# brucechin/OctopusZK

Hardware: AMD Instinct MI355X
Metric: BN254 G1 VariableBaseMSM Mscalar-mul/s at 2^20 (higher is better)
Workload: dtype u32; 1 GPU; VariableBaseMSM BN254 G1 2^20 random scalars/bases per GPU, bit-exact vs the serial CPU path (BASELINE.json configs[1]); n_per_gpu=1048576, window_bits=16, windows=8, glv=True, prepared_bases=False, msms_in_flight=3, schedule=pipeline3, parallelism=index-range shard x1, RCCL all-gather of 192-B partials + HIP point sum

## Files before the change

octopuszk_amd/csrc/ec_fft.cuh:

```cuda
#pragma once
#include "points_scale.cuh"

namespace ozk {

template <class CV>
OZK_HD void ec_write2(const Jac<CV>& a, const Jac<CV>& b, bool negate_b, u32* oa, u32* ob) {
  using IO = CurveIO<CV>;
  const bool ia = is_inf(a), ib = is_inf(b);
  if (ia || ib) {
    IO::template write<WireIn>(a, oa);
    if (ib) return IO::template write_inf<WireIn>(ob);
    return IO::template write_jac<WireIn>(b, inv(b.Z), negate_b, ob);
  }
  const auto za = reduce_to<32>(a.Z), zb = reduce_to<32>(b.Z);
  const auto ti = inv(mul(za, zb));
  IO::template write_jac<WireIn>(a, mul(ti, zb), false, oa);
  IO::template write_jac<WireIn>(b, mul(ti, za), negate_b, ob);
}
template <class CV>
OZK_HD Aff<typename CV::EA> ec_to_affine(const Jac<CV>& r) {
  using IO = CurveIO<CV>;
  using EA = typename CV::EA;
  Aff<EA> q = IO::aff_infinity();
  if (is_inf(r)) return q;
  q = IO::jac_to_aff(r, inv(r.Z));
  q.x = EA(canonical(q.x));
  q.y = EA(canonical(q.y));
  return q;
}
template <class EA>
OZK_HD Aff<EA> ec_neg(const Aff<EA>& q) {
  Aff<EA> m;
  m.x = q.x;
  m.y = EA(canonical(neg(q.y)));
  return m;
}

template <class CV>
OZK_HD void points_add_one(const u32* pa, const u32* pb, bool negate_b, u32* out) {
  using IO = CurveIO<CV>;
  const auto a = IO::aff_from_wire(pa);
  auto b = IO::aff_from_wire(pb);
  if (negate_b) b = ec_neg(b);
  IO::template write<WireIn>(jac_madd<CV>(from_affine<CV>(a), b), out);
}

struct EcFftTwiddle {
  u32 base[8], k[8];
};
OZK_HD void ecfft_twiddle(const EcFftTwiddle& c, u32 i, u32 (&out)[8]) {
  using F = Fe<FrParams, 32>;
  F acc = F(to_mont<FrParams>(c.k)), b = F(to_mont<FrParams>(c.base));
  for (u32 e = i; e; e >>= 1) {
    if (e & 1) acc = F(mul(acc, b));
    b = F(sqr(b));
  }
  from_mont(acc, out);
}
OZK_HD void ecfft_schedule(const EcFftTwiddle& c, u32 i, bool glv, ScaleSchedule& s) {
  u32 w[8];
  ecfft_twiddle(c, i, w);
  scale_recode(w, glv, s);
}

template <class CV, bool GLV>
OZK_HD void ecfft_butterfly(const u32* pa, const u32* pb, const ScaleSchedule* sa, const ScaleSchedule* sb, u32* oa,
                            u32* ob) {
  auto a = CurveIO<CV>::aff_from_wire(pa);
  const auto b = CurveIO<CV>::aff_from_wire(pb);
  if (sa) a = ec_to_affine<CV>(scale_ladder<CV, GLV>(a, *sa));
  const Jac<CV> v = sb ? scale_ladder<CV, GLV>(b, *sb) : from_affine<CV>(b);
  const Jac<CV> sum = jac_madd<CV>(v, a);
  const Jac<CV> dif = jac_madd<CV>(v, ec_neg(a));
  ec_write2<CV>(sum, dif, true, oa, ob);
}

OZK_HD bool words_are(const u32* w, const u32 (&v)[8]) {
  u32 d = 0;
  for (int i = 0; i < 8; i++) d |= w[i] ^ v[i];
  return d == 0;
}
template <class CV>
OZK_HD Jac<CV> sparse_term(const Jac<CV>& acc, const u32* p, const u32* c) {
  auto q = CurveIO<CV>::aff_from_wire(p);
  if (c) {
    u32 k[8];
    for (int i = 0; i < 8; i++) k[i] = c[i];
    for (int it = 0; it < 6 && mp_geq<8>(k, GlvConsts::R32); it++) mp_sub<8>(k, GlvConsts::R32);
    const u32 one[8] = {1, 0, 0, 0, 0, 0, 0, 0};
    u32 m1[8];
    for (int i = 0; i < 8; i++) m1[i] = GlvConsts::R32[i];
    m1[0] -= 1;
    if (words_are(k, m1)) {
      q = ec_neg(q);
    } else if (!words_are(k, one)) {
      const Jac<CV> v = is_inf(q) ? jac_infinity<CV>() : scalar_mul<CV>(q, k, 8);
      q = ec_to_affine<CV>(v);
    }
  }
  return jac_madd<CV>(acc, q);
}

#if defined(__HIPCC__)
constexpr int EC_LONG = 64;
constexpr int EC_LONG_LANES = 4096;

template <int TYPE>
__global__ __launch_bounds__(64) void k_ecfft_recode(EcFftTwiddle c, int n, ScaleSchedule* out) {
  const int i = blockIdx.x * blockDim.x + threadIdx.x;
  if (i >= n) return;
  ScaleSchedule s;
  ecfft_schedule(c, (u32)i, EcType<TYPE>::GLV, s);
  out[i] = s;
}

template <int TYPE>
__global__ __launch_bounds__(64) void k_ecfft_permute(const u32* __restrict__ in, int n, int logn, u32* __restrict__ out) {
  using CV = typename EcType<TYPE>::CV;
  using IO = CurveIO<CV>;
  constexpr int PW = IO::WIRE_JAC_WORDS;
  const int i = blockIdx.x * blockDim.x + threadIdx.x;
  if (i >= n) return;
  const u32 j = logn ? __brev((u32)i) >> (32 - logn) : 0u;
  IO::template write_aff<WireIn>(IO::aff_from_wire(in + (size_t)PW * i), out + (size_t)PW * j);
}

template <int TYPE>
__global__ __launch_bounds__(64) void k_ecfft_pass(u32* data, int logn, int logh, const ScaleSchedule* tab, int stride,
                                                   int skip0, const ScaleSchedule* sa) {
  using CV = typename EcType<TYPE>::CV;
  constexpr int PW = CurveIO<CV>::WIRE_JAC_WORDS;
  const u32 t = blockIdx.x * blockDim.x + threadIdx.x;
  if (t >= (1u << (logn - 1))) return;
  const int logb = logn - 1 - logh;
  const u32 j = t >> logb, k = t & ((1u << logb) - 1);
  u32* pa = data + (size_t)PW * (((size_t)k << (logh + 1)) + j);
  u32* pb = pa + ((size_t)PW << logh);
  const ScaleSchedule* sb = (j == 0 && skip0) ? nullptr : tab + (size_t)j * stride;
  ecfft_butterfly<CV, EcType<TYPE>::GLV>(pa, pb, sa, sb, pa, pb);
}

template <int TYPE>
__global__ __launch_bounds__(64) void k_points_add(const u32* a, const u32* b, int n, int negate_b, u32* out) {
  using CV = typename EcType<TYPE>::CV;
  constexpr int PW = CurveIO<CV>::WIRE_JAC_WORDS;
  const int i = blockIdx.x * blockDim.x + threadIdx.x;
  if (i >= n) return;
  points_add_one<CV>(a + (size_t)PW * i, b + (size_t)PW * i, negate_b != 0, out + (size_t)PW * i);
}

template <int TYPE>
__global__ __launch_bounds__(64) void k_sparse_points(const u32* __restrict__ ptr, const u32* __restrict__ idx,
                                                      const u32* __restrict__ coeff, const u32* __restrict__ points,
                                                      int rows, u32* __restrict__ out) {
  using CV = typename EcType<TYPE>::CV;
  using IO = CurveIO<CV>;
  constexpr int PW = IO::WIRE_JAC_WORDS;
  const int row = blockIdx.x * blockDim.x + threadIdx.x;
  if (row >= rows) return;
  const u32 b = ptr[row], e = ptr[row + 1];
  if (e - b > (u32)EC_LONG) return;
  Jac<CV> acc = jac_infinity<CV>();
  for (u32 t = b; t < e; t++)
    acc = sparse_term<CV>(acc, points + (size_t)PW * idx[t], coeff ? coeff + (size_t)8 * t : nullptr);
  IO::template write<WireIn>(acc, out + (size_t)PW * row);
}
template <int TYPE>
__global__ __launch_bounds__(64) void k_sparse_points_long(const u32* __restrict__ ptr, const u32* __restrict__ idx,
                                                           const u32* __restrict__ coeff, const u32* __restrict__ points,
                                                           const u32* __restrict__ long_rows, u32* __restrict__ part) {
  using CV = typename EcType<TYPE>::CV;
  using IO = CurveIO<CV>;
  constexpr int PW = IO::WIRE_JAC_WORDS;
  const u32 g = blockIdx.x * blockDim.x + threadIdx.x;
  const u32 lr = g / EC_LONG_LANES, l = g % EC_LONG_LANES;
  const u32 row = long_rows[lr];
  const u32 b = ptr[row], e = ptr[row + 1];
  Jac<CV> acc = jac_infinity<CV>();
  for (u32 t = b + l; t < e; t += EC_LONG_LANES)
    acc = sparse_term<CV>(acc, points + (size_t)PW * idx[t], coeff ? coeff + (size_t)8 * t : nullptr);
  IO::template write<WireIn>(acc, part + (size_t)PW * g);
}
template <int TYPE>
__global__ __launch_bounds__(64) void k_points_sum64(const u32* __restrict__ in, int groups, const u32* __restrict__ dest,
                                                     u32* __restrict__ out) {
  using CV = typename EcType<TYPE>::CV;
  using IO = CurveIO<CV>;
  constexpr int PW = IO::WIRE_JAC_WORDS;
  const int g = blockIdx.x * blockDim.x + threadIdx.x;
  if (g >= groups) return;
  Jac<CV> acc = jac_infinity<CV>();
  for (int i = 0; i < 64; i++) acc = jac_madd<CV>(acc, IO::aff_from_wire(in + (size_t)PW * (64 * (size_t)g + i)));
  IO::template write<WireIn>(acc, out + (size_t)PW * (dest ? dest[g] : (u32)g));
}
#endif

}
```

octopuszk_amd/csrc/glv.cuh:

```cuda
#pragma once
#include "curve.cuh"

namespace ozk {

struct GlvConsts {
  static constexpr u32 R32[8] = {0xf0000001u, 0x43e1f593u, 0x79b97091u, 0x2833e848u, 0x8181585du, 0xb85045b6u, 0xe131a029u, 0x30644e72u};
  static constexpr u32 G1C[3] = {0xc7e0b3d7u, 0xd91d232eu, 0x00000002u};
  static constexpr u32 G2C[5] = {0x391eb18du, 0x7a7bd9d4u, 0xa773d2cfu, 0x4ccef014u, 0x00000002u};
  static constexpr u32 A1[2] = {0x94d213e3u, 0x89d32568u};
  static constexpr u32 A2[4] = {0x1221250bu, 0x0be4e154u, 0xeeb859fdu, 0x6f4d8248u};
  static constexpr u32 B1ABS[4] = {0x7d4f1128u, 0x8211bbebu, 0xeeb859fcu, 0x6f4d8248u};
  static constexpr u32 B2[2] = {0x94d213e3u, 0x89d32568u};
  static constexpr u32 BETA_G1[9] = {0xa337995u, 0x158d1d23u, 0x189c9b98u, 0x12fa4e45u, 0x185faadcu, 0x176f16du, 0xeed93bau, 0x14291140u, 0xc0afeu};
  static constexpr u32 BETA_G2[9] = {0x18ccb791u, 0x175b1c3au, 0xb83d6e2u, 0xe8ed071u, 0x1282bee2u, 0x4220e84u, 0x1fe4017fu, 0x15084d4au, 0x169119u};
};

template <int NA, int NB, int NR>
OZK_HD void mp_mul_lo(const u32* a, const u32* b, u32* r) {
  u64 carry = 0;
#pragma unroll
  for (int k = 0; k < NR; k++) {
    u64 lo = carry & 0xffffffffull;
    u64 hi = carry >> 32;
#pragma unroll
    for (int i = 0; i < NA; i++) {
      const int j = k - i;
      if (j >= 0 && j < NB) {
        const u64 p = (u64)a[i] * b[j];
        lo += p & 0xffffffffull;
        hi += p >> 32;
      }
    }
    r[k] = (u32)lo;
    carry = hi + (lo >> 32);
  }
}
template <int NA, int NB>
OZK_HD void mp_mul(const u32* a, const u32* b, u32* r) { mp_mul_lo<NA, NB, NA + NB>(a, b, r); }

template <int N>
OZK_HD void mp_sub(u32* a, const u32* b) {
  u64 br = 0;
#pragma unroll
  for (int i = 0; i < N; i++) {
    const u64 t = (u64)a[i] - b[i] - br;
    a[i] = (u32)t;
    br = (t >> 32) & 1;
  }
}
template <int N>
OZK_HD bool mp_geq(const u32* a, const u32* b) {
  for (int i = N - 1; i >= 0; i--) {
    if (a[i] > b[i]) return true;
    if (a[i] < b[i]) return false;
  }
  return true;
}
template <int N>
OZK_HD void mp_neg(u32* a) {
  u64 c = 1;
#pragma unroll
  for (int i = 0; i < N; i++) {
    c += (u64)(~a[i]);
    a[i] = (u32)c;
    c >>= 32;
  }
}

OZK_HD void glv_decompose(const u32 (&k_in)[8], u32 (&k1)[4], bool& neg1, u32 (&k2)[4], bool& neg2) {
  u32 k[8];
#pragma unroll
  for (int i = 0; i < 8; i++) k[i] = k_in[i];
  for (int it = 0; it < 6 && mp_geq<8>(k, GlvConsts::R32); it++) mp_sub<8>(k, GlvConsts::R32);
  u32 p1[11], p2[13];
  mp_mul<8, 3>(k, GlvConsts::G1C, p1);
  mp_mul<8, 5>(k, GlvConsts::G2C, p2);
  const u32* c1 = p1 + 8;
  const u32* c2 = p2 + 8;
  u32 t1[5], t2[5], s1[5], s2[5];
  mp_mul_lo<3, 2, 5>(c1, GlvConsts::A1, t1);
  mp_mul_lo<5, 4, 5>(c2, GlvConsts::A2, t2);
#pragma unroll
  for (int i = 0; i < 5; i++) s1[i] = k[i];
  mp_sub<5>(s1, t1);
  mp_sub<5>(s1, t2);
  mp_mul_lo<3, 4, 5>(c1, GlvConsts::B1ABS, s2);
  mp_mul_lo<5, 2, 5>(c2, GlvConsts::B2, t2);
  mp_sub<5>(s2, t2);
  neg1 = (s1[4] >> 31) != 0;
  neg2 = (s2[4] >> 31) != 0;
  if (neg1) mp_neg<5>(s1);
  if (neg2) mp_neg<5>(s2);
#pragma unroll
  for (int i = 0; i < 4; i++) {
    k1[i] = s1[i];
    k2[i] = s2[i];
  }
}

template <class CV>
OZK_HD Fe<FqParams, 16> glv_beta() {
  if constexpr (CurveIO<CV>::CW == 16) return fe_const<FqParams, 16>(GlvConsts::BETA_G2);
  else return fe_const<FqParams, 16>(GlvConsts::BETA_G1);
}
template <class CV>
OZK_HD Aff<typename CV::EA> glv_image(const Aff<typename CV::EA>& q) {
  Aff<typename CV::EA> q2;
  q2.x = typename CV::EA(canonical(scale(q.x, glv_beta<CV>())));
  q2.y = q.y;
  return q2;
}

}
```

octopuszk_amd/csrc/msm_var.cuh:

```cuda
#pragma once
#include "curve.cuh"
#include "glv.cuh"

namespace ozk {

constexpr u32 BID_NONE = 0xffffffffu;

struct MsmPlan {
  int n_in;
  int glv;
  int n;
  int sd;
  int c;
  int cb;
  int W;
  int L1;
  int LK;
  int S;
};

OZK_HD u32 scalar_digit(const u32 (&s)[8], int w, int c) {
  const int bit = w * c;
  const int wi = bit >> 5, sh = bit & 31;
  u32 v = s[wi] >> sh;
// ... 859 lines not shown
    const long long e0 = (s + L < n_in) ? (s + L) : n_in;
    bool any = false;
    for (long long p = s; p < e0; p++) any = any || (bid_in[p] != BID_NONE);
    live = any;
  }
  if (live) {
    const long long e = (s + L < n_in) ? (s + L) : n_in;
    const u32 first_bid = bid_at(s);
    const bool cb = (s > 0) && (bid_at(s - 1) == first_bid) && (first_bid != BID_NONE);
    const u32 last_bid = bid_at(e - 1);
    const bool cf = (e < n_in) && (bid_at(e) == last_bid) && (last_bid != BID_NONE);
    u32 cur = BID_NONE;
    bool cur_cb = false;
    using Acc = std::conditional_t<(FIRST && CV::LDS_ACC), RunAccLds<CV>, RunAcc<CV, FIRST>>;
    Acc acc;
    if constexpr (FIRST && CV::LDS_ACC) {
      extern __shared__ u32 ozk_acc_lds[];
      acc.init(ozk_acc_lds);
    }
    if constexpr (FIRST) {
      const u32 n_e = (u32)(e - s);
      const uint2* ent_c = ent + s;
      const uint2 e_first = ent_c[0];
      uint2 e_next = ent_c[n_e > 1 ? 1 : 0];
      u32 v_cur = e_first.x;
      const __amdgpu_buffer_rsrc_t table = Acc::table_rsrc(pts_in);
      typename Acc::Raw r = Acc::load_raw_buf(table, v_cur);
      u32 b_cur = first_bid;
      for (u32 k = 0; k < n_e; k++) {
        const u32 b = b_cur;
        const bool negate = (v_cur & SIDX_NEG) != 0;
        const auto q = [&] {
          if constexpr (LAZY) return Acc::decode_unsigned(r);
          else return Acc::decode(r, v_cur);
        }();
        const u32 k2 = (k + 2 < n_e) ? k + 2 : n_e - 1;
        const uint2 en = e_next;
        r = Acc::load_raw_buf(table, en.x);
        b_cur = en.y;
        v_cur = en.x;
        e_next = ent_c[k2];
        if (b != cur) {
          if (cur != BID_NONE) {
            if (cur_cb) {
              head_bid = cur;
              acc.store(pts_out + (size_t)(2 * (size_t)t) * IO::REC_WORDS);
            } else {
              acc.store(buckets + (size_t)cur * IO::REC_WORDS);
            }
          }
          cur = b;
          cur_cb = (k == 0) && cb;
          if constexpr (LAZY) acc.start_signed(q, negate);
          else acc.start_q(q);
        } else {
          if constexpr (LAZY) acc.accumulate_signed(q, negate);
          else acc.accumulate_q(q);
        }
      }
    } else {
    for (long long p = s; p < e; p++) {
      const u32 b = bid_in[p];
      if (b != cur) {
        if (cur != BID_NONE) {
          if (cur_cb) {
            head_bid = cur;
            acc.store(pts_out + (size_t)(2 * (size_t)t) * IO::REC_WORDS);
          } else {
            acc.store(buckets + (size_t)cur * IO::REC_WORDS);
          }
        }
        cur = b;
        cur_cb = (p == s) && cb;
        if (b != BID_NONE) acc.start(pts_in, idx_in, p);
      } else if (b != BID_NONE) {
        acc.accumulate(pts_in, idx_in, p);
      }
    }
    }
    if (cur != BID_NONE) {
      if (cur_cb) {
        head_bid = cur;
        acc.store(pts_out + (size_t)(2 * (size_t)t) * IO::REC_WORDS);
        if (cf) {
          tail_bid = cur;
          if constexpr (FIRST) {
            acc.store_infinity(pts_out + (size_t)(2 * (size_t)t + 1) * IO::REC_WORDS);
          } else {
            IO::store_rec_jac(jac_infinity<CV>(), pts_out + (size_t)(2 * (size_t)t + 1) * IO::REC_WORDS);
          }
        }
      } else if (cf) {
        tail_bid = cur;
        acc.store(pts_out + (size_t)(2 * (size_t)t + 1) * IO::REC_WORDS);
      } else {
        acc.store(buckets + (size_t)cur * IO::REC_WORDS);
      }
    }
  }
  bid_out[2 * (size_t)t] = head_bid;
  bid_out[2 * (size_t)t + 1] = tail_bid;
}

template <class CV, bool FIRST, bool LAZY = false>
__global__ void __launch_bounds__(256, (FIRST && CV::LDS_ACC) ? 2 : 1)
k_segreduce(const u32* __restrict__ bid_in, const u32* __restrict__ idx_in, const u32* __restrict__ pts_in,
            const u32* __restrict__ d_count, int n_in_static, int L,
            u32* __restrict__ buckets, u32* __restrict__ bid_out, u32* __restrict__ pts_out,
            int n_lanes, unsigned long long* __restrict__ clk) {
  const int t = blockIdx.x * blockDim.x + threadIdx.x;
  unsigned long long w0 = 0, c0 = 0;
  if constexpr (FIRST) {
    if (clk != nullptr && threadIdx.x == 0) {
      w0 = (unsigned long long)wall_clock64();
      c0 = (unsigned long long)clock64();
      atomicMax(&clk[0], ~w0);
    }
  }
  if (t < n_lanes)
    segreduce_lane<CV, FIRST, LAZY>(t, bid_in, idx_in, pts_in, d_count, n_in_static, L, buckets, bid_out, pts_out);
  if constexpr (FIRST) {
    if (clk != nullptr && (threadIdx.x & 63) == 0) {
      const unsigned long long w1 = (unsigned long long)wall_clock64();
      atomicMax(&clk[1], w1);
      if (threadIdx.x == 0) {
        atomicAdd(&clk[2], (unsigned long long)clock64() - c0);
        atomicAdd(&clk[3], w1 - w0);
      }
    }
  }
}

static __global__ void k_read_clock(unsigned long long* out) { out[0] = (unsigned long long)wall_clock64(); }

template <class CV>
__global__ void __launch_bounds__(256)
k_segreduce_small(const u32* __restrict__ d_count, int n_in, int L, u32* __restrict__ buckets,
                  u32* __restrict__ bid_a, u32* __restrict__ pts_a, u32* __restrict__ bid_b, u32* __restrict__ pts_b) {
  if (*d_count == 0) return;
  u32 *bi = bid_a, *pi = pts_a, *bo = bid_b, *po = pts_b;
  while (true) {
    const int lanes = (n_in + L - 1) / L;
    for (int t = threadIdx.x; t < lanes; t += blockDim.x)
      segreduce_lane<CV, false>(t, bi, nullptr, pi, d_count, n_in, L, buckets, bo, po);
    if (lanes == 1) break;
    block_sync();
    n_in = 2 * lanes;
    u32* tb = bi; bi = bo; bo = tb;
    u32* tp = pi; pi = po; po = tp;
  }
}

constexpr int RUN_MAX = 16;
template <class CV>
__global__ void __launch_bounds__(256)
k_runmerge(const u32* __restrict__ bid_in, const u32* __restrict__ pts, int n_slots,
           u32* __restrict__ buckets, u32* __restrict__ bid_out, u32* __restrict__ remaining) {
  using IO = CurveIO<CV>;
  const int t = blockIdx.x * blockDim.x + threadIdx.x;
  u32 alive = 0;
#pragma unroll 1
  for (int k = 0; k < 2; k++) {
    const int x = 2 * t + 1 + k;
    if (x >= n_slots) break;
    const u32 bx = bid_in[x];
    u32 out = BID_NONE;
    if (bx != BID_NONE) {
      int s = x, e = x;
      while (s > 0 && x - s < RUN_MAX && bid_in[s - 1] == bx) s--;
      while (e + 1 < n_slots && e - x < RUN_MAX && bid_in[e + 1] == bx) e++;
      const bool is_short = (x - s < RUN_MAX) && (e - x < RUN_MAX) && (e - s + 1 <= RUN_MAX);
      if (!is_short) {
        out = bx;
      } else if (s == x) {
        Xyzz<CV> acc = IO::load_xyzz(pts + (size_t)s * IO::REC_WORDS);
        for (int q = s + 1; q <= e; q += 2) acc = xyzz_add(acc, IO::load_xyzz(pts + (size_t)q * IO::REC_WORDS));
        IO::store_rec_xyzz(acc, buckets + (size_t)bx * IO::REC_WORDS);
      }
    }
    bid_out[x] = out;
    alive += (out != BID_NONE);
  }
  if (t == 0 && n_slots > 0) {
    bid_out[0] = bid_in[0];
    alive += (bid_in[0] != BID_NONE);
  }
  for (int o = 32; o > 0; o >>= 1) alive += __shfl_xor(alive, o);
  if ((threadIdx.x & 63) == 0 && alive) atomicAdd(remaining, alive);
}

template <class CV, bool FIRSTLEVEL>
__global__ void __launch_bounds__(256)
k_wsum(const u32* __restrict__ A_in, const u32* __restrict__ R_in, const u32* __restrict__ hist,
       int m_in, int S, int g, u32* __restrict__ A_out, u32* __restrict__ R_out, int m_out, int W, int prio) {
  using IO = CurveIO<CV>;
  if (prio) __builtin_amdgcn_s_setprio(3);
  const int t = blockIdx.x * blockDim.x + threadIdx.x;
  if (t >= m_out * W) return;
  const int w = t / m_out, j = t - w * m_out;
  const size_t base = (size_t)w * m_in;
  const int lo = j * S;
  int hi = lo + S;
  if (hi > m_in) hi = m_in;
  Jac<CV> run = jac_infinity<CV>(), ws = jac_infinity<CV>(), asum = jac_infinity<CV>();
  for (int e = hi - 1; e >= lo; e--) {
    if constexpr (FIRSTLEVEL) {
      if (hist[base + e] != 0) run = jac_add(run, IO::load_rec(R_in + (base + e) * IO::REC_WORDS));
    } else {
      run = jac_add(run, IO::load_jac(R_in + (base + e) * IO::JAC_WORDS));
    }
    if (e > lo) ws = jac_add(ws, run);
    if constexpr (!FIRSTLEVEL) asum = jac_add(asum, IO::load_jac(A_in + (base + e) * IO::JAC_WORDS));
  }
  for (int k = 0; k < g; k++) ws = jac_dbl(ws);
  if constexpr (!FIRSTLEVEL) ws = jac_add(ws, asum);
  IO::store_jac(ws, A_out + ((size_t)w * m_out + j) * IO::JAC_WORDS);
  IO::store_jac(run, R_out + ((size_t)w * m_out + j) * IO::JAC_WORDS);
}

template <class CV>
__device__ __forceinline__ Jac<CV> shfl_down_jac(const Jac<CV>& p, int o) {
  Jac<CV> r;
  r.X = shfl_down_el(p.X, o);
  r.Y = shfl_down_el(p.Y, o);
  r.Z = shfl_down_el(p.Z, o);
  return r;
}

template <class CV>
__device__ __forceinline__ void wave_combine(Jac<CV>& A, Jac<CV>& T, int l, int valid, int g) {
  for (int o = 1; o < valid; o <<= 1) {
    const Jac<CV> t = shfl_down_jac(T, o);
    const Jac<CV> s = jac_add(T, t);
    if (l + o < 64) T = s;
  }
  Jac<CV> U = T;
  for (int k = 0; k < g; k++) U = jac_dbl(U);
  const Jac<CV> AV = jac_add(A, U);
  Jac<CV> V = (l >= 1) ? AV : A;
  int top = 1;
  while (top < valid) top <<= 1;
  for (int o = top >> 1; o > 0; o >>= 1) {
    const Jac<CV> v = shfl_down_jac(V, o);
    const Jac<CV> s = jac_add(V, v);
    if (l < o) V = s;
  }
  A = V;
}

template <class CV>
__global__ void __launch_bounds__(64)
k_wsum_wave(const u32* __restrict__ A_in, const u32* __restrict__ R_in, int m_in, int g,
            u32* __restrict__ A_out, u32* __restrict__ R_out, int m_out, int W) {
  using IO = CurveIO<CV>;
  __builtin_amdgcn_s_setprio(3);
  const int wave = blockIdx.x;
  if (wave >= m_out * W) return;
  const int w = wave / m_out, j = wave - w * m_out;
  const int l = threadIdx.x & 63;
  const int e = j * 64 + l;
  int valid = m_in - j * 64;
  if (valid > 64) valid = 64;
  Jac<CV> A = jac_infinity<CV>(), T = jac_infinity<CV>();
  if (e < m_in) {
    A = IO::load_jac(A_in + ((size_t)w * m_in + e) * IO::JAC_WORDS);
    T = IO::load_jac(R_in + ((size_t)w * m_in + e) * IO::JAC_WORDS);
  }
  wave_combine<CV>(A, T, l, valid, g);
  if (l == 0) {
    IO::store_jac(A, A_out + ((size_t)w * m_out + j) * IO::JAC_WORDS);
    IO::store_jac(T, R_out + ((size_t)w * m_out + j) * IO::JAC_WORDS);
  }
}

template <class CV>
__global__ void __launch_bounds__(64)
k_wsum_fused(const u32* __restrict__ buckets, const u32* __restrict__ hist, int m_in, int S, int sg,
             u32* __restrict__ A_out, u32* __restrict__ R_out, int m_out, int W, int prio) {
  using IO = CurveIO<CV>;
  if (prio) __builtin_amdgcn_s_setprio(3);
  const int wave = blockIdx.x;
  if (wave >= m_out * W) return;
  const int w = wave / m_out, j = wave - w * m_out;
  const int l = threadIdx.x & 63;
  const int nseg = (m_in + S - 1) / S;
  int valid = nseg - j * 64;
  if (valid > 64) valid = 64;
  const size_t base = (size_t)w * m_in;
  const int lo = (j * 64 + l) * S;
  int hi = lo + S;
  if (hi > m_in) hi = m_in;
  Jac<CV> run = jac_infinity<CV>(), ws = jac_infinity<CV>();
  for (int e = hi - 1; e >= lo; e--) {
    if (hist[base + e] != 0) run = jac_add(run, IO::load_rec(buckets + (base + e) * IO::REC_WORDS));
    if (e > lo) ws = jac_add(ws, run);
  }
  wave_combine<CV>(ws, run, l, valid, sg);
  if (l == 0) {
    IO::store_jac(ws, A_out + ((size_t)w * m_out + j) * IO::JAC_WORDS);
    IO::store_jac(run, R_out + ((size_t)w * m_out + j) * IO::JAC_WORDS);
  }
}

struct SliceBuckets {
  const u32* buckets[16];
  const u32* hist[16];
};
template <class CV>
__global__ void __launch_bounds__(256) k_bucket_combine(SliceBuckets t, int K, u32* __restrict__ buckets0,
                                                        u32* __restrict__ hist0, size_t NB) {
  using IO = CurveIO<CV>;
  const size_t e = (size_t)blockIdx.x * blockDim.x + threadIdx.x;
  if (e >= NB) return;
  bool have = hist0[e] != 0, changed = false;
  Jac<CV> acc = jac_infinity<CV>();
  if (have) acc = IO::load_rec(buckets0 + e * IO::REC_WORDS);
  for (int k = 1; k < K; k++) {
    if (t.hist[k][e] == 0) continue;
    acc = jac_add(acc, IO::load_rec(t.buckets[k] + e * IO::REC_WORDS));
    changed = true;
  }
  if (changed) {
    IO::store_rec_jac(acc, buckets0 + e * IO::REC_WORDS);
    hist0[e] = 1;
  }
}

template <class CV>
__device__ __forceinline__ void write_normalised_inline(const Jac<CV>& r, u32* out) {
  CurveIO<CV>::template write<WireOut>(r, out);
}
template <class CV>
__device__ void write_normalised(const Jac<CV>& r, u32* out) {
  write_normalised_inline<CV>(r, out);
}

template <class CV>
__global__ void __launch_bounds__(64) k_finalize(const u32* __restrict__ A_w, const u32* __restrict__ R_w, int m,
                                                 int g, int W, int c, int sd, u32* __restrict__ out) {
  using IO = CurveIO<CV>;
  __shared__ u32 sw[64 * IO::JAC_WORDS];
// ... 132 lines not shown
```

octopuszk_amd/csrc/msm_var_driver.cuh:

```cuda
#pragma once
#include <hip/hip_ext.h>
#include <pthread.h>
#include <stdlib.h>

#include <atomic>
#include <vector>

#include "msm_var.cuh"
#include "host_ctx.h"
#include "fq2.cuh"

namespace ozk {

enum { PROF_OFF = 0, PROF_EVENTS = 1, PROF_CLOCK = 2 };
struct ProfState {
  pthread_mutex_t mu = PTHREAD_MUTEX_INITIALIZER;
  std::atomic<int> mode{PROF_OFF};
  int src = PROF_EVENTS;
  int every = 1, seen = 0;
  int count = 0;
  std::vector<hipEvent_t> e0, e1;
  bool created = false;
  int ev_device = -1;
  unsigned long long* d_clk = nullptr;
// ... 233 lines not shown
enum { TAIL_LATENCY = 0, TAIL_THROUGHPUT = 1 };
struct TailShape {
  bool fused;
  int serial_above;
};
static TailShape tail_shape(int mode) {
  const int forced = env_int("OZK_MSM_TAIL_MODE", -1);
  if (forced == 0 || forced == 1) mode = forced;
  TailShape t;
  t.fused = env_int("OZK_MSM_WSUM_FUSED", mode == TAIL_THROUGHPUT ? 0 : 1) != 0;
  t.serial_above = env_int("OZK_MSM_TAIL_SERIAL_ABOVE", mode == TAIL_THROUGHPUT ? 64 : (1 << 30));
  return t;
}
static void first_level_shape(const MsmPlan& p, bool fused, int* m_out, int* g_out) {
  const int m_in = 1 << p.cb;
  const int nseg = (m_in + p.S - 1) / p.S;
  const int sg = ilog2((uint32_t)p.S);
  if (fused) {
    *m_out = (nseg + 63) / 64;
    *g_out = sg + 6;
  } else {
    *m_out = nseg;
    *g_out = sg;
  }
}
template <class CV>
void launch_wsum0(const MsmPlan& p, const MsmLayout& L, hipStream_t st, int prio, bool fused) {
  const int TB = 256;
  const int m_in = 1 << p.cb;
  int m_out, g;
  first_level_shape(p, fused, &m_out, &g);
  const int tot = m_out * p.W;
  if (fused)
    hipLaunchKernelGGL((k_wsum_fused<CV>), dim3(tot), dim3(64), 0, st, L.buckets, L.hist_t, m_in, p.S,
                       ilog2((uint32_t)p.S), L.wA[0], L.wR[0], m_out, p.W, prio);
  else
    hipLaunchKernelGGL((k_wsum<CV, true>), dim3((tot + TB - 1) / TB), dim3(TB), 0, st, (const u32*)nullptr,
                       L.buckets, L.hist_t, m_in, p.S, 0, L.wA[0], L.wR[0], m_out, p.W, prio);
}

template <class CV>
int var_msm_sort(const void* d_bases, const void* d_scalars, int n, void* sorted, size_t sorted_bytes,
                        void* sort_ws, size_t sort_ws_bytes, hipStream_t st, hipEvent_t order_ev = nullptr,
                        const void* prepared = nullptr) {
  hip_clear_stale();
  const MsmPlan p = plan_for<CV>(n);
  if (prepared && p.glv && !p.sd) return fail(OZK_E_INVALID, "prepared bases need the signed-digit plan");
  RegionBytes rb;
  const MsmLayout L = make_layout3<CV>(p, sorted, sort_ws, nullptr, &rb, prepared);
  if (rb.sorted > sorted_bytes || rb.sort_ws > sort_ws_bytes)
    return fail(OZK_E_INVALID, "sort buffers too small: need %zu + %zu bytes, got %zu + %zu", rb.sorted, rb.sort_ws,
                sorted_bytes, sort_ws_bytes);
  const int TB = 256;
  const u32* bases = (const u32*)d_bases;
  const u32* scalars = (const u32*)d_scalars;
  const int n_in = p.n_in;
  n = p.n;
  OZK_HIP(hipMemsetAsync(L.total, 0, 4 * sizeof(u32), st));
  if (p.glv) {
    hipLaunchKernelGGL(k_digits_glv, dim3((n_in + TB - 1) / TB), dim3(TB), 0, st, scalars, n_in, p.c, p.W, p.sd,
                       L.digits, L.neg_flags);
    if (!prepared)
      hipLaunchKernelGGL((k_convert_bases<CV>), dim3((n_in + TB - 1) / TB), dim3(TB), 0, st, bases, L.aff, n_in, 1,
                         p.sd ? (const uint8_t*)nullptr : (const uint8_t*)L.neg_flags);
  } else {
    if (!prepared)
      hipLaunchKernelGGL((k_convert_bases<CV>), dim3((n_in + TB - 1) / TB), dim3(TB), 0, st, bases, L.aff, n_in, 0,
                         (const uint8_t*)nullptr);
    hipLaunchKernelGGL(k_digits, dim3((n_in + TB - 1) / TB), dim3(TB), 0, st, scalars, n_in, p.c, p.W, L.digits);
  }
  if (n <= SORTS_MAX_N && p.cb <= SORTS_MAX_CB && env_int("OZK_MSM_SMALL_SORT", 1)) {
    hipLaunchKernelGGL(k_sort_small, dim3(p.W), dim3(SORTS_BLOCK), 0, st, L.digits, n, p.cb, p.sd, L.total, L.hist, L.sent);
    if (order_ev && env_int("OZK_MSM_ORDER", 1)) OZK_HIP(hipStreamWaitEvent(st, order_ev, 0));
    OZK_HIP(hipGetLastError());
    return OZK_OK;
  }
  const size_t lds1 = (size_t)L.NH * sizeof(u32);
  hipLaunchKernelGGL(k_sort1_count, dim3(L.nblk, p.W), dim3(SORT_BLOCK), lds1, st, L.digits, n, L.lo_bits, p.sd,
                     L.NH, L.nblk, L.C1);
  const int items = SCAN_BLOCK * SCAN_ITEMS;
  const int nb = (int)((L.nC1 + items - 1) / items);
  hipLaunchKernelGGL(k_scan_blocksum, dim3(nb), dim3(SCAN_BLOCK), 0, st, L.C1, (int)L.nC1, L.blocksum);
  hipLaunchKernelGGL(k_scan_top, dim3(1), dim3(1024), 0, st, L.blocksum, nb, L.total);
  hipLaunchKernelGGL(k_scan_final, dim3(nb), dim3(SCAN_BLOCK), 0, st, L.C1, (int)L.nC1, L.blocksum, L.P1);
  const size_t lds_sc = ((size_t)2 * L.NH + 2 * SORT_CHUNK) * sizeof(u32);
  hipLaunchKernelGGL(k_sort1_scatter, dim3(L.nblk, p.W), dim3(SORT_BLOCK), lds_sc, st, L.digits, n, L.lo_bits,
                     p.sd, L.NH, L.nblk, L.P1, L.total, L.nC1, L.coarse);
  const int nbins = p.W * L.NH;
  const u32 sign_bit = p.sd ? 0x80u : 0u;
  const u32 big_thresh = (u32)(n / 64) > SORT_BIG ? (u32)(n / 64) : SORT_BIG;
  if (L.cap / ((size_t)big_thresh + 1) > (size_t)SORTBIG_MAXBINS)
    return fail(OZK_E_INVALID, "window plan c=%d (W=%d) at n=%d can produce more than %d oversized sort bins",
                p.c, p.W, p.n_in, SORTBIG_MAXBINS);
  hipLaunchKernelGGL(k_sort2, dim3(nbins), dim3(SORT2_BLOCK), 0, st, L.coarse, L.P1, L.total, p.cb, L.lo_bits, L.NH,
                     sign_bit, L.nblk, nbins, big_thresh, L.hist, L.sent);
  if (order_ev && env_int("OZK_MSM_ORDER", 1)) OZK_HIP(hipStreamWaitEvent(st, order_ev, 0));
  hipLaunchKernelGGL(k_sortbig_list, dim3(1), dim3(256), 0, st, L.P1, L.total, L.nblk, nbins, big_thresh, L.bigbins);
  hipLaunchKernelGGL(k_sortbig_count, dim3(1024), dim3(SORT_BLOCK), 0, st, L.coarse, L.bigbins,
                     (1u << L.lo_bits) - 1u, L.bigT);
  hipLaunchKernelGGL(k_sortbig_scan, dim3(SORTBIG_MAXBINS), dim3(256), 0, st, L.bigbins, L.bigT, p.cb, L.lo_bits, L.NH,
                     L.hist);
  hipLaunchKernelGGL(k_sortbig_scatter, dim3(1024), dim3(SORT_BLOCK), 0, st, L.coarse, L.bigbins, L.bigT, p.cb,
                     L.lo_bits, sign_bit, L.NH, L.sent);
  OZK_HIP(hipGetLastError());
  return OZK_OK;
}

enum { ACCUM_ALL = 0, ACCUM_LEVEL1 = 1, ACCUM_REST = 2 };
template <class CV>
int var_msm_accum(int n, void* sorted, size_t sorted_bytes, void* accum_ws, size_t accum_ws_bytes, void* tail,
                         size_t tail_bytes, hipStream_t st, const void* prepared = nullptr, int part = ACCUM_ALL) {
  hip_clear_stale();
  using CT = CV;
  const MsmPlan p = plan_for<CV>(n);
  RegionBytes rb;
  MsmLayout L = make_layout3<CV>(p, sorted, nullptr, accum_ws, &rb, prepared);
  if (rb.sorted > sorted_bytes || rb.accum_ws > accum_ws_bytes)
    return fail(OZK_E_INVALID, "accumulate buffers too small: need %zu + %zu bytes, got %zu + %zu", rb.sorted,
                rb.accum_ws, sorted_bytes, accum_ws_bytes);
  const size_t tneed = tail_layout<CV>(p, L, tail, tail_bytes);
  if (tneed > tail_bytes) return fail(OZK_E_INVALID, "tail buffer too small: need %zu bytes, got %zu", tneed, tail_bytes);
  const int TB = 256;
  size_t lanes = (L.cap + p.L1 - 1) / p.L1;
  if (part != ACCUM_REST) {
  hipEvent_t prof_e0 = nullptr, prof_e1 = nullptr;
  unsigned long long* clk = nullptr;
  g_prof.claim(&prof_e0, &prof_e1, &clk);
  const bool prof = prof_e0 != nullptr;
  size_t acc_lds = CV::LDS_ACC ? (size_t)RunAccLds<CV>::LDS_WORDS * TB * sizeof(u32) : 0;
  if (!CV::LDS_ACC) acc_lds = (size_t)env_int("OZK_L1_LDS", 41216);
  auto launch_l1 = [&](auto kern) {
    if (acc_lds > 65536)
      OZK_HIP(hipFuncSetAttribute((const void*)kern, hipFuncAttributeMaxDynamicSharedMemorySize, (int)acc_lds));
    hipExtLaunchKernelGGL(kern, dim3((unsigned)((lanes + TB - 1) / TB)), dim3(TB), (uint32_t)acc_lds, st,
                          prof ? prof_e0 : (hipEvent_t) nullptr, prof ? prof_e1 : (hipEvent_t) nullptr, 0u,
                          (const u32*)nullptr, (const u32*)L.sent, (const u32*)L.aff, (const u32*)L.total, 0, p.L1,
                          L.buckets, L.slot_bid[0], L.slot_pts[0], (int)lanes, clk);
    return OZK_OK;
  };
  int rc_l1;
  if constexpr (CV::LAZY_MADD) {
    if (env_int("OZK_L1_LAZY", 1)) rc_l1 = launch_l1(k_segreduce<CV, true, true>);
    else rc_l1 = launch_l1(k_segreduce<CV, true, false>);
  } else {
    rc_l1 = launch_l1(k_segreduce<CV, true, false>);
  }
  if (rc_l1) return rc_l1;
  }
  if (part == ACCUM_LEVEL1) {
    OZK_HIP(hipGetLastError());
    return OZK_OK;
  }
  size_t n_in = 2 * lanes;
  hipLaunchKernelGGL((k_runmerge<CT>), dim3((unsigned)((lanes + TB - 1) / TB)), dim3(TB), 0, st, L.slot_bid[0],
                     L.slot_pts[0], (int)n_in, L.buckets, L.slot_bid2, L.total + 1);
  int cur = 0;
  bool first_generic = true;
  const int small_lanes = env_int("OZK_MSM_SMALL_LEVEL_LANES", 1024);
  while (true) {
    lanes = (n_in + p.LK - 1) / p.LK;
    if (!first_generic && (int)lanes <= small_lanes) {
      hipLaunchKernelGGL((k_segreduce_small<CT>), dim3(1), dim3(TB), 0, st, L.total + 1, (int)n_in, p.LK, L.buckets,
                         L.slot_bid[cur], L.slot_pts[cur], L.slot_bid[cur ^ 1], L.slot_pts[cur ^ 1]);
      break;
    }
    hipLaunchKernelGGL((k_segreduce<CT, false>), dim3((unsigned)((lanes + TB - 1) / TB)), dim3(TB), 0, st,
                       first_generic ? L.slot_bid2 : L.slot_bid[cur], (const u32*)nullptr, L.slot_pts[cur],
                       L.total + 1, (int)n_in, p.LK, L.buckets, L.slot_bid[cur ^ 1], L.slot_pts[cur ^ 1], (int)lanes,
                       (unsigned long long*)nullptr);
    first_generic = false;
    if (lanes == 1) break;
    n_in = 2 * lanes;
    cur ^= 1;
  }
  OZK_HIP(hipMemcpyAsync(L.hist_t, L.hist, L.NB * sizeof(u32), hipMemcpyDeviceToDevice, st));
  OZK_HIP(hipGetLastError());
  return OZK_OK;
}

template <class CV>
int var_msm_head(const void* d_bases, const void* d_scalars, int n, void* ws, size_t ws_bytes, void* tail,
                        size_t tail_bytes, hipStream_t st, hipEvent_t order_ev = nullptr,
                        const void* prepared = nullptr) {
  const RegionBytes rb = region_bytes<CV>(n);
  if (rb.sorted + rb.sort_ws + rb.accum_ws > ws_bytes)
    return fail(OZK_E_INVALID, "workspace too small: need %zu bytes, got %zu", rb.sorted + rb.sort_ws + rb.accum_ws,
                ws_bytes);
  uint8_t* w = (uint8_t*)ws;
  int rc = var_msm_sort<CV>(d_bases, d_scalars, n, w, rb.sorted, w + rb.sorted, rb.sort_ws, st, order_ev, prepared);
  if (rc) return rc;
  return var_msm_accum<CV>(n, w, rb.sorted, w + rb.sorted + rb.sort_ws, rb.accum_ws, tail, tail_bytes, st, prepared);
}

template <class CV>
int var_msm_tail(int n, void* tail, size_t tail_bytes, void* d_out, hipStream_t st,
                        hipEvent_t order_ev = nullptr, int mode = TAIL_LATENCY) {
  hip_clear_stale();
  using CT = CV;
  MsmPlan p = plan_for<CV>(n);
  MsmLayout L;
  L.m1 = (((size_t)1 << p.cb) + p.S - 1) / p.S;
  const size_t tneed = tail_layout<CV>(p, L, tail, tail_bytes);
  if (tneed > tail_bytes) return fail(OZK_E_INVALID, "tail buffer too small: need %zu bytes, got %zu", tneed, tail_bytes);
  const TailShape shape = tail_shape(mode);
  if (shape.fused && mode == TAIL_LATENCY) {
    int s_dflt = p.S;
    if (std::is_same<CV, G1Cfg>::value && p.cb >= 13) s_dflt = 8;
    const int s_lat = env_int("OZK_MSM_S_LAT", s_dflt);
    if (s_lat >= 2 && s_lat <= 64) p.S = 1 << ilog2((uint32_t)s_lat);
  }
  launch_wsum0<CV>(p, L, st, env_int("OZK_MSM_WSUM0_PRIO", 0), shape.fused);
  int m_in, g, k = 0;
  first_level_shape(p, shape.fused, &m_in, &g);
  const int TB = 256;
  const int sg = ilog2((uint32_t)p.S);
  const int serial_above = shape.serial_above < 1 ? 1 : shape.serial_above;
  while (m_in > serial_above) {
    const int m_out = (m_in + p.S - 1) / p.S;
    const int tot = m_out * p.W;
    hipLaunchKernelGGL((k_wsum<CT, false>), dim3((tot + TB - 1) / TB), dim3(TB), 0, st, L.wA[k], L.wR[k],
                       (const u32*)nullptr, m_in, p.S, g, L.wA[k ^ 1], L.wR[k ^ 1], m_out, p.W, 1);
    m_in = m_out;
    g += sg;
    k ^= 1;
  }
  int fin_max = env_int("OZK_MSM_FIN_MAX", 4);
  if (fin_max < 1) fin_max = 1;
  if (fin_max > 16) fin_max = 16;
  const bool order_early = env_int("OZK_MSM_ORDER_EARLY", 1) != 0;
  if (order_ev && order_early) OZK_HIP(hipEventRecord(order_ev, st));
  while (m_in > fin_max) {
    const int m_out = (m_in + 63) / 64;
    const int tot = m_out * p.W;
    hipLaunchKernelGGL((k_wsum_wave<CT>), dim3(tot), dim3(64), 0, st, L.wA[k], L.wR[k], m_in, g, L.wA[k ^ 1],
                       L.wR[k ^ 1], m_out, p.W);
    m_in = m_out;
    g += 6;
    k ^= 1;
  }
  if (order_ev && !order_early) OZK_HIP(hipEventRecord(order_ev, st));
  hipLaunchKernelGGL((k_finalize<CT>), dim3(1), dim3(64), 0, st, L.wA[k], L.wR[k], m_in, g, p.W, p.c, p.sd,
                     (u32*)d_out);
  OZK_HIP(hipGetLastError());
  return OZK_OK;
}

template <class CV>
size_t var_msm_tail_bytes(int n) {
  const MsmPlan p = plan_for<CV>(n);
  MsmLayout L;
  L.m1 = (((size_t)1 << p.cb) + p.S - 1) / p.S;
  return tail_layout<CV>(p, L, nullptr, 0);
}

template <class CV>
int var_msm_dev(const void* d_bases, const void* d_scalars, int n, void* d_out, void* ws,
                       size_t ws_bytes, hipStream_t st, const void* prepared = nullptr) {
  LonePlan lone;
  const RegionBytes rb0 = region_bytes<CV>(n);
  const size_t main_bytes = rb0.sorted + rb0.sort_ws + rb0.accum_ws;
  const size_t tb = var_msm_tail_bytes<CV>(n);
  if (main_bytes + tb > ws_bytes)
    return fail(OZK_E_INVALID, "workspace too small: need %zu bytes, got %zu", main_bytes + tb, ws_bytes);
  uint8_t* tail = (uint8_t*)ws + main_bytes;
  int rc = var_msm_head<CV>(d_bases, d_scalars, n, ws, main_bytes, tail, tb, st, nullptr, prepared);
  if (rc) return rc;
  return var_msm_tail<CV>(n, tail, tb, d_out, st);
}

template <class CV>
size_t var_msm_head_ws_bytes(int n) {
  const RegionBytes rb = region_bytes<CV>(n);
  return rb.sorted + rb.sort_ws + rb.accum_ws;
}
template <class CV>
size_t var_msm_ws_bytes(int n) {
  return var_msm_head_ws_bytes<CV>(n) + var_msm_tail_bytes<CV>(n);
}

inline int host_slices(int n) {
  int kmax = env_int("OZK_HOST_SLICES", 8);
  if (kmax > MAX_SLICES) kmax = MAX_SLICES;
  int min_log = env_int("OZK_HOST_SLICE_MIN_LOG", 18);
  if (min_log < 4) min_log = 4;
  if (min_log > 30) min_log = 30;
  int k = n >> min_log;
  if (k > kmax) k = kmax;
  return k < 1 ? 1 : k;
}

inline int host_slice_per(int n, int K) {
  if (K < 2) return n;
  if (env_int("OZK_HOST_SLICE_TAPER", 1) == 0) return (n + K - 1) / K;
  const long long rest = (long long)n - (long long)n / (2 * K);
  return (int)((rest + K - 2) / (K - 1));
}
static bool plans_agree(int n1, int n2) {
  const MsmPlan a = make_plan(n1), b = make_plan(n2);
  return a.c == b.c && a.cb == b.cb && a.W == b.W && a.sd == b.sd && a.glv == b.glv && a.S == b.S;
}

template <class CV>
size_t host_sliced_ws_bytes(int K, int per) {
  return pad256(var_msm_head_ws_bytes<CV>(per)) + (size_t)K * pad256(var_msm_tail_bytes<CV>(per));
}
template <class CV>
int host_sliced_msm(HostCtx* c, const uint8_t* bases, const uint8_t* scalars, int n, int K, int per, uint8_t* d_bases,
                    uint8_t* d_sc, uint8_t* d_ws, uint8_t* d_out, hipEvent_t* ev, hipStream_t st, hipStream_t up) {
  hip_clear_stale();
  using IO = CurveIO<CV>;
  const size_t base_rec = (size_t)IO::WIRE_JAC_WORDS * 4;
  const size_t padded = (size_t)K * per;
  const size_t main_bytes = pad256(var_msm_head_ws_bytes<CV>(per));
  const size_t tb = pad256(var_msm_tail_bytes<CV>(per));
  uint8_t* d_tails = d_ws + main_bytes;
  int rc;
  const long long last_ns = (long long)n - (long long)(K - 1) * per;
  if (last_ns < 1) return fail(OZK_E_INTERNAL, "slice plan: %d slices of %d pairs exceed n = %d", K, per, n);
  const bool exact_last = last_ns < per && plans_agree(per, (int)last_ns);
  if (padded > (size_t)n && !exact_last) {
    if (scalars) OZK_HIP(hipMemsetAsync(d_sc + (size_t)n * 32, 0, (padded - n) * 32, up));
    OZK_HIP(hipMemsetAsync(d_bases + (size_t)n * base_rec, 0, (padded - n) * base_rec, up));
  }
  const MsmPlan p = plan_for<CV>(per);
  SliceBuckets sb = {};
  for (int s = 0; s < K; s++) {
    const size_t lo = (size_t)s * per;
    const size_t ns = ((size_t)n - lo < (size_t)per) ? ((size_t)n - lo) : (size_t)per;
// ... 193 lines not shown
```

Measured before the change: 719.5 Mscalar-mul/s.

## Streamline GLV decomposition, rebalance runmerge work lists, fold histogram copy into kernel

Replaces the iterative subtract loop for scalar reduction mod r with a single quotient-estimate subtraction plus one conditional subtract. It also narrows the GLV multiprecision products to the limbs actually needed and makes the final negation branchless. In k_runmerge, short-run accumulation for non-LDS curves is split into per-round work items distributed across the block through shared memory, to reduce divergence from serial per-thread loops. The separate device-to-device histogram memcpy is folded into the runmerge kernel, adding a grid-stride copy and a block sync at kernel start.

```diff
diff --git a/octopuszk_amd/csrc/ec_fft.cuh b/octopuszk_amd/csrc/ec_fft.cuh
--- a/octopuszk_amd/csrc/ec_fft.cuh
+++ b/octopuszk_amd/csrc/ec_fft.cuh
@@ -86,7 +86,7 @@
   if (c) {
     u32 k[8];
     for (int i = 0; i < 8; i++) k[i] = c[i];
-    for (int it = 0; it < 6 && mp_geq<8>(k, GlvConsts::R32); it++) mp_sub<8>(k, GlvConsts::R32);
+    reduce_mod_r(k);
     const u32 one[8] = {1, 0, 0, 0, 0, 0, 0, 0};
     u32 m1[8];
     for (int i = 0; i < 8; i++) m1[i] = GlvConsts::R32[i];
diff --git a/octopuszk_amd/csrc/glv.cuh b/octopuszk_amd/csrc/glv.cuh
--- a/octopuszk_amd/csrc/glv.cuh
+++ b/octopuszk_amd/csrc/glv.cuh
@@ -17,26 +17,22 @@
 
 template <int NA, int NB, int NR>
 OZK_HD void mp_mul_lo(const u32* a, const u32* b, u32* r) {
-  u64 carry = 0;
 #pragma unroll
-  for (int k = 0; k < NR; k++) {
-    u64 lo = carry & 0xffffffffull;
-    u64 hi = carry >> 32;
+  for (int k = 0; k < NR; k++) r[k] = 0;
+#pragma unroll
+  for (int j = 0; j < NB; j++) {
+    u32 carry = 0;
 #pragma unroll
     for (int i = 0; i < NA; i++) {
-      const int j = k - i;
-      if (j >= 0 && j < NB) {
-        const u64 p = (u64)a[i] * b[j];
-        lo += p & 0xffffffffull;
-        hi += p >> 32;
+      if (i + j < NR) {
+        const u64 t = mad64(a[i], b[j], (u64)r[i + j] + carry);
+        r[i + j] = (u32)t;
+        carry = (u32)(t >> 32);
       }
     }
-    r[k] = (u32)lo;
-    carry = hi + (lo >> 32);
+    if (NA + j < NR) r[NA + j] = carry;
   }
 }
-template <int NA, int NB>
-OZK_HD void mp_mul(const u32* a, const u32* b, u32* r) { mp_mul_lo<NA, NB, NA + NB>(a, b, r); }
 
 template <int N>
 OZK_HD void mp_sub(u32* a, const u32* b) {
@@ -57,40 +53,65 @@
   return true;
 }
 template <int N>
-OZK_HD void mp_neg(u32* a) {
-  u64 c = 1;
+OZK_HD void mp_cneg(u32* a, bool neg) {
+  const u32 m = 0u - (u32)neg;
+  u64 c = m & 1u;
 #pragma unroll
   for (int i = 0; i < N; i++) {
-    c += (u64)(~a[i]);
+    c += (u64)(a[i] ^ m);
     a[i] = (u32)c;
     c >>= 32;
   }
+}
+
+OZK_HD void reduce_mod_r(u32 (&k)[8]) {
+  const u32 q = k[7] / (GlvConsts::R32[7] + 1u);
+  u64 m = 0;
+  u32 br = 0;
+#pragma unroll
+  for (int i = 0; i < 8; i++) {
+    m = mad64(q, GlvConsts::R32[i], m);
+    const u64 t = (u64)k[i] - (u32)m - br;
+    k[i] = (u32)t;
+    br = (u32)(t >> 32) & 1u;
+    m >>= 32;
+  }
+  u32 d[8];
+  br = 0;
+#pragma unroll
+  for (int i = 0; i < 8; i++) {
+    const u64 t = (u64)k[i] - GlvConsts::R32[i] - br;
+    d[i] = (u32)t;
+    br = (u32)(t >> 32) & 1u;
+  }
+#pragma unroll
+  for (int i = 0; i < 8; i++) k[i] = br ? k[i] : d[i];
 }
 
 OZK_HD void glv_decompose(const u32 (&k_in)[8], u32 (&k1)[4], bool& neg1, u32 (&k2)[4], bool& neg2) {
   u32 k[8];
 #pragma unroll
   for (int i = 0; i < 8; i++) k[i] = k_in[i];
-  for (int it = 0; it < 6 && mp_geq<8>(k, GlvConsts::R32); it++) mp_sub<8>(k, GlvConsts::R32);
-  u32 p1[11], p2[13];
-  mp_mul<8, 3>(k, GlvConsts::G1C, p1);
-  mp_mul<8, 5>(k, GlvConsts::G2C, p2);
+  reduce_mod_r(k);
+  u32 p1[10], p2[12];
+  mp_mul_lo<8, 3, 10>(k, GlvConsts::G1C, p1);
+  mp_mul_lo<8, 5, 12>(k, GlvConsts::G2C, p2);
   const u32* c1 = p1 + 8;
   const u32* c2 = p2 + 8;
-  u32 t1[5], t2[5], s1[5], s2[5];
-  mp_mul_lo<3, 2, 5>(c1, GlvConsts::A1, t1);
-  mp_mul_lo<5, 4, 5>(c2, GlvConsts::A2, t2);
+  u32 t1[4], t2[4], s1[4], s2[4];
+  mp_mul_lo<2, 2, 4>(c1, GlvConsts::A1, t1);
+  mp_mul_lo<4, 4, 4>(c2, GlvConsts::A2, t2);
 #pragma unroll
-  for (int i = 0; i < 5; i++) s1[i] = k[i];
-  mp_sub<5>(s1, t1);
-  mp_sub<5>(s1, t2);
-  mp_mul_lo<3, 4, 5>(c1, GlvConsts::B1ABS, s2);
-  mp_mul_lo<5, 2, 5>(c2, GlvConsts::B2, t2);
-  mp_sub<5>(s2, t2);
-  neg1 = (s1[4] >> 31) != 0;
-  neg2 = (s2[4] >> 31) != 0;
-  if (neg1) mp_neg<5>(s1);
-  if (neg2) mp_neg<5>(s2);
+  for (int i = 0; i < 4; i++) s1[i] = k[i];
+  mp_sub<4>(s1, t1);
+  mp_sub<4>(s1, t2);
+  mp_mul_lo<2, 4, 4>(c1, GlvConsts::B1ABS, s2);
+  mp_mul_lo<4, 2, 4>(c2, GlvConsts::B2, t2);
+  mp_sub<4>(s2, t2);
+  neg1 = (s1[3] >> 31) != 0;
+  neg2 = (s2[3] >> 31) != 0;
+  mp_cneg<4>(s1, neg1);
+  mp_cneg<4>(s2, neg2);
 #pragma unroll
   for (int i = 0; i < 4; i++) {
     k1[i] = s1[i];
diff --git a/octopuszk_amd/csrc/msm_var.cuh b/octopuszk_amd/csrc/msm_var.cuh
--- a/octopuszk_amd/csrc/msm_var.cuh
+++ b/octopuszk_amd/csrc/msm_var.cuh
@@ -1035,12 +1035,23 @@
 }
 
 constexpr int RUN_MAX = 16;
-template <class CV>
-__global__ void __launch_bounds__(256)
+constexpr int RUNMERGE_BLOCK = 256;
+template <class CV>
+__global__ void __launch_bounds__(RUNMERGE_BLOCK)
 k_runmerge(const u32* __restrict__ bid_in, const u32* __restrict__ pts, int n_slots,
-           u32* __restrict__ buckets, u32* __restrict__ bid_out, u32* __restrict__ remaining) {
+           u32* __restrict__ buckets, u32* __restrict__ bid_out, u32* __restrict__ remaining,
+           const u32* __restrict__ hist_src, u32* __restrict__ hist_dst, size_t n_hist) {
   using IO = CurveIO<CV>;
+  constexpr bool LIST = !CV::LDS_ACC;
+  constexpr int ROUNDS = RUN_MAX / 2;
+  constexpr int CAP = 2 * RUNMERGE_BLOCK;
+  __shared__ u32 item_s[2][CAP];
+  __shared__ uint8_t item_span[2][CAP];
+  __shared__ u32 item_cnt[ROUNDS + 1];
+  if (threadIdx.x <= ROUNDS) item_cnt[threadIdx.x] = 0;
   const int t = blockIdx.x * blockDim.x + threadIdx.x;
+  for (size_t i = (size_t)t; i < n_hist; i += (size_t)gridDim.x * blockDim.x) hist_dst[i] = hist_src[i];
+  block_sync();
   u32 alive = 0;
 #pragma unroll 1
   for (int k = 0; k < 2; k++) {
@@ -1056,9 +1067,17 @@
       if (!is_short) {
         out = bx;
       } else if (s == x) {
-        Xyzz<CV> acc = IO::load_xyzz(pts + (size_t)s * IO::REC_WORDS);
-        for (int q = s + 1; q <= e; q += 2) acc = xyzz_add(acc, IO::load_xyzz(pts + (size_t)q * IO::REC_WORDS));
-        IO::store_rec_xyzz(acc, buckets + (size_t)bx * IO::REC_WORDS);
+        if constexpr (!LIST) {
+          Xyzz<CV> acc = IO::load_xyzz(pts + (size_t)s * IO::REC_WORDS);
+          for (int q = s + 1; q <= e; q += 2) acc = xyzz_add(acc, IO::load_xyzz(pts + (size_t)q * IO::REC_WORDS));
+          IO::store_rec_xyzz(acc, buckets + (size_t)bx * IO::REC_WORDS);
+        } else if (e > s) {
+          const u32 j = atomicAdd(&item_cnt[0], 1u);
+          item_s[0][j] = (u32)s;
+          item_span[0][j] = (uint8_t)(e - s);
+        } else {
+          IO::store_rec_xyzz(IO::load_xyzz(pts + (size_t)s * IO::REC_WORDS), buckets + (size_t)bx * IO::REC_WORDS);
+        }
       }
     }
     bid_out[x] = out;
@@ -1070,6 +1089,28 @@
   }
   for (int o = 32; o > 0; o >>= 1) alive += __shfl_xor(alive, o);
   if ((threadIdx.x & 63) == 0 && alive) atomicAdd(remaining, alive);
+#pragma unroll 1
+  for (int r = 0; LIST && r < ROUNDS; r++) {
+    block_sync();
+    const u32 len = (u32)__builtin_amdgcn_readfirstlane((int)item_cnt[r]);
+    if (len == 0) break;
+    const int cur = r & 1;
+#pragma unroll 1
+    for (u32 i = threadIdx.x; i < len; i += RUNMERGE_BLOCK) {
+      const u32 s = item_s[cur][i];
+      const u32 span = item_span[cur][i];
+      u32* bucket = buckets + (size_t)bid_in[s] * IO::REC_WORDS;
+      const u32 off = 2u * (u32)r + 1u;
+      const u32* sum = r == 0 ? pts + (size_t)s * IO::REC_WORDS : bucket;
+      const Xyzz<CV> acc = xyzz_add(IO::load_xyzz(sum), IO::load_xyzz(pts + ((size_t)s + off) * IO::REC_WORDS));
+      IO::store_rec_xyzz(acc, bucket);
+      if (off + 2u <= span) {
+        const u32 j = atomicAdd(&item_cnt[r + 1], 1u);
+        item_s[cur ^ 1][j] = s;
+        item_span[cur ^ 1][j] = (uint8_t)span;
+      }
+    }
+  }
 }
 
 template <class CV, bool FIRSTLEVEL>
diff --git a/octopuszk_amd/csrc/msm_var_driver.cuh b/octopuszk_amd/csrc/msm_var_driver.cuh
--- a/octopuszk_amd/csrc/msm_var_driver.cuh
+++ b/octopuszk_amd/csrc/msm_var_driver.cuh
@@ -409,8 +409,9 @@
     return OZK_OK;
   }
   size_t n_in = 2 * lanes;
+  static_assert(RUNMERGE_BLOCK == 256, "k_runmerge's work list is sized for this launch");
   hipLaunchKernelGGL((k_runmerge<CT>), dim3((unsigned)((lanes + TB - 1) / TB)), dim3(TB), 0, st, L.slot_bid[0],
-                     L.slot_pts[0], (int)n_in, L.buckets, L.slot_bid2, L.total + 1);
+                     L.slot_pts[0], (int)n_in, L.buckets, L.slot_bid2, L.total + 1, (const u32*)L.hist, L.hist_t, L.NB);
   int cur = 0;
   bool first_generic = true;
   const int small_lanes = env_int("OZK_MSM_SMALL_LEVEL_LANES", 1024);
@@ -430,7 +431,6 @@
     n_in = 2 * lanes;
     cur ^= 1;
   }
-  OZK_HIP(hipMemcpyAsync(L.hist_t, L.hist, L.NB * sizeof(u32), hipMemcpyDeviceToDevice, st));
   OZK_HIP(hipGetLastError());
   return OZK_OK;
 }
```

Result: faster. 729.5 Mscalar-mul/s, median of 6 (+1.4%).
